# NVIDIA/cuopt

Measured on NVIDIA H100. Metric: pdlp_iterations_per_sec, higher is better.
Workload: dtype f64

## Files before the change

### cuopt_b200/csrc/pdlp_kernels.cuh

```cuda
#pragma once

#include "device_utils.cuh"
#include "spmv_bicsr.cuh"

#include <math_constants.h>

namespace cuopt_b200 {

constexpr int EW_THREADS  = 256;
static __device__ int g_l2_hints = 1;

struct pdhg_ctl_t {
  double step_size, primal_weight, tau, sigma;
  double pending_weight;
  double sum_weights;
  double interaction, norm_dx2, norm_dy2;
  double reduction_exponent, growth_exponent, primal_smoothing, dual_smoothing;
  int parity;
  int pending_avg;
  int active;
  int valid;
  int k_pdhg;
  int attempts;
  int accepted;
// ... 645 lines not shown
    dy2 += __ldcg(scal + 4 * g + 2);
  }
  pdhg_step_rule(ctl, interaction, dx2, dy2);
}

template <int FMT = 0>
__global__ void __launch_bounds__(BICSR_THREADS, BICSR_MIN_CTAS) k_block_pass(const pdhg_ctl_t* __restrict__ ctl,
                                                                              bicsr_view_t Ab,
                                                                              const double* __restrict__ x0,
                                                                              const double* __restrict__ x1,
                                                                              int pick_candidate,
                                                                              double* __restrict__ t,
                                                                              int first,
                                                                              const unsigned long long* wait_flags,
                                                                              int n_wait)
{
  if (!ctl->active) return;
  __shared__ double rows[BICSR_WARPS][BICSR_SLOTS];
  if (wait_flags) peer_wait(wait_flags, n_wait, (unsigned long long)ctl->attempts + 1ull);
  const double* x       = pick_candidate ? (ctl->parity ? x0 : x1) : x0;
  const l2_policy_t pol = make_l2_policies(g_l2_hints);
  struct payload_t {
    double init;
  };
  auto pre_op = [&](int r) {
    payload_t p;
    p.init = first ? 0.0 : ld_l2(t + r, pol.stream);
    return p;
  };
  auto row_op = [&](int r, double s, const payload_t&) { st_l2(t + r, s, pol.stream); };
  spmv_bicsr_rows<payload_t, true, 1, FMT>(Ab, x, rows[threadIdx.x >> 5], pre_op, row_op, pol.keep);
}

__global__ void __launch_bounds__(EW_THREADS) k_flush_average(const pdhg_ctl_t* __restrict__ ctl,
                                                              int n,
                                                              const double* __restrict__ xbuf0,
                                                              const double* __restrict__ xbuf1,
                                                              double* __restrict__ sum_x,
                                                              int m,
                                                              const double* __restrict__ ybuf0,
                                                              const double* __restrict__ ybuf1,
                                                              double* __restrict__ sum_y)
{
  if (!ctl->pending_avg) return;
  const int cur    = ctl->parity;
  const double* x  = cur ? xbuf1 : xbuf0;
  const double* y  = cur ? ybuf1 : ybuf0;
  const double w   = ctl->pending_weight;
  const int stride = gridDim.x * blockDim.x;
  for (int j = blockIdx.x * blockDim.x + threadIdx.x; j < n; j += stride) sum_x[j] = sum_x[j] + w * x[j];
  for (int i = blockIdx.x * blockDim.x + threadIdx.x; i < m; i += stride) sum_y[i] = sum_y[i] + w * y[i];
}
__global__ void k_clear_pending(pdhg_ctl_t* ctl) { ctl->pending_avg = 0; }
__global__ void k_begin_batch(pdhg_ctl_t* ctl, int steps)
{
  ctl->target = ctl->accepted + steps;
  ctl->valid  = 0;
  ctl->active = steps > 0 ? 1 : 0;
}

__global__ void __launch_bounds__(BICSR_THREADS, BICSR_MIN_CTAS) k_spmv(bicsr_view_t A,
                                                                        const double* __restrict__ x,
                                                                        double* __restrict__ out)
{
  __shared__ double rows[BICSR_WARPS][BICSR_SLOTS];
  struct payload_t {};
// ... 569 lines not shown
```

### cuopt_b200/csrc/pdlp_solver.cu

```cuda
#include "pdlp_solver.hpp"

#include "dist_comm.hpp"
#include "pdlp_kernels.cuh"
#include "presolve.cuh"
#include "trust_region.cuh"

#include <math_constants.h>
#include <nvtx3/nvToolsExt.h>

#include <algorithm>
#include <chrono>
#include <cmath>
#include <cstdio>
#include <cstdlib>
#include <atomic>
#include <map>
#include <mutex>
#include <thread>
#include <string>

namespace cuopt_b200 {

namespace {

// ... 31 lines not shown
    structure = &o;
    val.copy_from(o.val, s);
  }
};

constexpr int SCHEDULE_SEGMENT = 1 << 16;
template <typename T, typename F>
std::vector<T> cut_in_segments(int rows, F cut_segment)
{
  const int n_seg = std::max(1, (rows + SCHEDULE_SEGMENT - 1) / SCHEDULE_SEGMENT);
  std::vector<std::vector<T>> part(n_seg);
  const int n_thr = (int)std::max(1u, std::min<unsigned>({std::thread::hardware_concurrency(), 32u, (unsigned)n_seg}));
  std::atomic<int> next{0};
  auto work = [&]() {
    for (int sgm = next.fetch_add(1); sgm < n_seg; sgm = next.fetch_add(1))
      cut_segment(sgm * SCHEDULE_SEGMENT, std::min(rows, (sgm + 1) * SCHEDULE_SEGMENT), part[sgm]);
  };
  if (n_thr <= 1) {
    work();
  } else {
    std::vector<std::thread> pool;
    for (int t = 0; t < n_thr; ++t) pool.emplace_back(work);
    for (auto& t : pool) t.join();
  }
  size_t total = 0;
  for (auto& v : part) total += v.size();
  std::vector<T> all;
  all.reserve(total + 1);
  for (auto& v : part) all.insert(all.end(), v.begin(), v.end());
  return all;
}

template <typename VI>
void build_bicsr(csr_dev_t& d, const VI& off, cudaStream_t s, int sms)
{
  const int all_rows = (int)off.size() - 1;
  constexpr int LONG = (int)0x80000000u;
  std::vector<int2> cut = cut_in_segments<int2>(all_rows, [&](int r, int rows, std::vector<int2>& out) {
    while (r < rows) {
      const int lo = off[r];
      if (off[r + 1] - lo > BICSR_SLOTS) {
        out.push_back(make_int2(r | LONG, r + 1));
        ++r;
        continue;
      }
      int r1 = r;
      while (r1 < rows && off[r1 + 1] - lo <= BICSR_SLOTS && (r1 - r) < BICSR_MAX_ROWS) ++r1;
      out.push_back(make_int2(r, r1));
      r = r1;
    }
  });
  std::vector<int2> desc;
  desc.reserve(cut.size());
  for (const int2& c : cut)
    if (!(c.x & LONG)) desc.push_back(c);
  const int n_std = (int)desc.size();
  for (const int2& c : cut)
    if (c.x & LONG) desc.push_back(make_int2(c.x & ~LONG, c.y));
  bicsr_dev_t& b = d.bi;
  b.n_std        = n_std;
  b.n_blk        = (int)desc.size();
  b.desc.upload(desc, s);
  b.row_slot.resize((size_t)std::max(all_rows, 1));
  b.idx.resize((size_t)std::max(n_std, 1) * BICSR_SLOTS);
  b.val.resize((size_t)std::max(n_std, 1) * BICSR_SLOTS);
  if (all_rows > 0) CUOPT_CUDA_TRY(cudaMemsetAsync(b.row_slot.data(), 0xff, (size_t)all_rows * sizeof(unsigned short), s));
  if (n_std > 0) {
    const int grid = std::max(1, std::min((n_std + 7) / 8, sms * 8));
    k_bicsr_fill<<<grid, 256, 0, s>>>(n_std, b.desc.data(), d.off.data(), d.idx.data(), d.val.data(), b.idx.data(),
                                      b.val.data(), b.row_slot.data());
    CUOPT_CUDA_TRY(cudaGetLastError());
  }
}
void fill_bicsr_values(csr_dev_t& d, cudaStream_t s, int sms)
{
  const bicsr_dev_t& st = d.bi_structure();
  d.bi.val.resize((size_t)std::max(st.n_std, 1) * BICSR_SLOTS);
  if (st.n_std > 0) {
    const int grid = std::max(1, std::min((st.n_std + 7) / 8, sms * 8));
    k_bicsr_fill_values<<<grid, 256, 0, s>>>(st.n_std, st.desc.data(), d.off_ptr(), d.val.data(), d.bi.val.data());
    CUOPT_CUDA_TRY(cudaGetLastError());
  }
}

void compact_bicsr(csr_dev_t& d, int fmt, int col0, cudaStream_t s, int sms)
{
  bicsr_dev_t& b = d.bi;
  b.fmt  = fmt;
  b.col0 = col0;
  if (fmt == 0 || b.n_std == 0) return;
  const size_t ns = (size_t)b.n_std;
  if (fmt & BICSR_FMT_IDX3) {
    b.lo16.resize(ns * BICSR_SLOTS);
    b.hi8.resize(ns * 32);
  }
  if (fmt & BICSR_FMT_MASK) b.mask.resize(ns * 8);
  const int grid = std::max(1, std::min((b.n_std + BICSR_WARPS - 1) / BICSR_WARPS, sms * 8));
  k_bicsr_fill_structure<<<grid, BICSR_THREADS, 0, s>>>(b.n_std, b.desc.data(), d.off.data(), d.idx.data(), col0,
                                                        b.lo16.data(), b.hi8.data(), b.mask.data());
  CUOPT_CUDA_TRY(cudaGetLastError());
  CUOPT_CUDA_TRY(cudaStreamSynchronize(s));
  if (fmt & BICSR_FMT_IDX3) b.idx = dvec<int>{};
  if (fmt & BICSR_FMT_MASK) b.row_slot = dvec<unsigned short>{};
}

// ... 129 lines not shown
  cudaEvent_t free_[SLOTS] = {};
  bool ensure()
  {
    if (tried_) return buf_ != nullptr;
    tried_ = true;
    if (cudaMallocHost(&buf_, SLOT * SLOTS) != cudaSuccess) {
      cudaGetLastError();
      buf_ = nullptr;
      return false;
    }
    for (auto& e : free_) cudaEventCreateWithFlags(&e, cudaEventDisableTiming);
    return true;
  }
};
template <typename T, typename V>
void upload_staged(dvec<T>& d, const V& h, cudaStream_t s)
{
  d.resize(h.size());
  staged_uploader_t::get().upload(d.data(), h.data(), h.size() * sizeof(T), s);
}
template <typename VI, typename VD>
void upload_csr(csr_dev_t& d, int rows, int cols, const VI& off, const VI& idx, const VD& val, cudaStream_t s, int sms)
{
  d.rows = rows;
  d.cols = cols;
  d.nnz  = (int)val.size();
  upload_staged(d.off, off, s);
  upload_staged(d.idx, idx, s);
  upload_staged(d.val, val, s);
  build_bicsr(d, off, s, sms);
}

constexpr double GATHER_BLOCK_L2_FRACTION = 0.32;

}

struct pdlp_solver_t::impl_t {
  int m = 0, n = 0, nnz = 0;
  bool maximize    = false;
  double obj_scale = 1.0, obj_offset = 0.0;
  pdlp_hyper_params_t hp;
  pdlp_settings_t st;
  cudaStream_t stream = nullptr;
  int sms             = 132;

  csr_dev_t A, AT, As, ATs;
  dvec<double> c, l, u, lc, uc, cs, ls, us, lcs, ucs, Dr, Dc;
  dvec<double> xbuf[2], ybuf[2], atybuf[2], xbar, sum_x, sum_y, x_avg, y_avg, x_lr, y_lr, rc_cur, rc_avg;
  dvec<double> part_dy2, part_k3, part_rows, part_cols, part_misc, scratch_n, scratch_m, d_scalar;
  dvec<double> dist_buf;
  const dist_context_t* dist = nullptr;
  bool sharded() const { return dist != nullptr && dist->world > 1; }
  bool dist_gather = false;
  int row0[DIST_MAX_PEERS + 1] = {};
  int m_total = 0;
  dvec<double> yfull, t_slice;
  void* yfull_peer[DIST_MAX_PEERS] = {};
  peer_ptrs_t p_yfull{};
  csr_dev_t ATslice;
  csr_dev_t Ahot;
  dvec<int> sendX, sendY;
  dvec<int> listX, listY;
  send_plan_t planX{}, planY{};
  dvec<double> xloc;
  int cntX = 0, cntY = 0;
  bool dist_pack = true;
// ... 28 lines not shown
  void* scal_peer[DIST_MAX_PEERS]  = {};
  void* flag_peer[DIST_MAX_PEERS]  = {};
  bool peers_open = false;
  peer_ptrs_t p_xbar{}, p_scal{};
  peer_flags_t p_flags{};
  dvec<unsigned> d_ticket;
  dvec<pdhg_ctl_t> d_ctl;
  dvec<eval_t> d_eval;
  pdhg_ctl_t* h_ctl = nullptr;
  eval_t* h_eval    = nullptr;
  double* h_scalar  = nullptr;
  int occ_spmv = 1;
  int occ_spmv2 = 1;
  int npre_override = 0;
  int compact_blocks = BICSR_FMT_IDX3 | BICSR_FMT_MASK;
  dvec<double> eval_m, eval_n;
  dvec<double> part_max;
  dvec<double> part_infeas;
  bool tr_enabled = false;
  double tr_gap_reduction_last_trial = 1.0;
  int grid_tr = 1;
  dvec<double> tr_aty, tr_ax, tr_grad, tr_dir, tr_thr, tr_thr_sorted, tr_A, tr_B, tr_parts, tr_scal;
  dvec<int> tr_iota, tr_perm;
  struct tr_gap_t {
    const double *px, *py;
    double pd = 0, dd = 0, dist = 0, lower = 0, upper = 0, ngap = 0;
  };
  struct gather_blocks_t {
    int B = 1, width = 0;
    int fmt = 0;
    std::vector<csr_dev_t> blk;
    std::vector<csr_dev_t> unscaled;
    std::vector<int> grid;
    bool on() const { return B > 1; }
  };
  gather_blocks_t blkA, blkAT, blkATslice;
  dvec<double> t_m, t_n;
  size_t gather_block_bytes = 0;
  int n_part_dy2 = 1;
  int grid_k1 = 1, grid_k2 = 1, grid_k3 = 1, grid_n = 1, grid_m = 1, grid_misc = 1;
  long long staged_fills = 0;
  std::map<int, cudaGraphExec_t> graphs;
  bool use_graphs = true;
  cudaEvent_t ev_a = nullptr, ev_b = nullptr;

  int total_pdlp_iterations      = 0;
  bool initialised               = false;
  bool need_aty                  = true;
  bool last_restart_was_average  = false;
  bool warm_started              = false;
  double last_candidate_kkt      = 0.0, last_restart_kkt = 0.0;
  double l2_norm_b = 0.0, l2_norm_c = 0.0;
  lp_solution_t sol;
  bool finished   = false;
  bool presolved    = false;
  bool postsolved   = false;
  presolve_state_t ps;
  double t_start  = 0.0;
  long long launches = 0;

  void close_peer_memory(bool collective)
  {
    if (!peers_open) return;
    cudaStreamSynchronize(stream);
    dist->close_peers(xbar_peer);
    dist->close_peers(scal_peer);
    dist->close_peers(flag_peer);
    dist->close_peers(yfull_peer);
    peers_open = false;
    if (collective) {
      dist->allreduce(d_scalar.data(), 1, true, stream);
// ... 173 lines not shown
    size_t pad = 0;
    if (sharded()) {
      if (dist->world > DIST_MAX_PEERS) throw lp_error(error_type_t::ValidationError, "at most 8 ranks per solve");
      nslice   = (((n + dist->world - 1) / dist->world) + 31) & ~31;
      n_pad    = nslice * dist->world;
      slice_j0 = std::min(n, dist->rank * nslice);
      slice_n  = std::max(0, std::min(nslice, n - slice_j0));
      pad      = (size_t)(n_pad - n);
    }
    for (int b = 0; b < 2; ++b) {
      xbuf[b].resize(n, pad); xbuf[b].zero(stream);
      ybuf[b].resize(m); ybuf[b].zero(stream);
      atybuf[b].resize(n, pad); atybuf[b].zero(stream);
    }
    xbar.resize(n, pad + (sharded() ? 64 * (size_t)dist->world + 64 : 0));
    xbar.zero(stream);
    sum_x.resize(n, pad);
    sum_x.zero(stream);
    for (dvec<double>* v : {&x_avg, &x_lr, &rc_cur, &rc_avg, &scratch_n}) { v->resize(n); v->zero(stream); }
    for (dvec<double>* v : {&sum_y, &y_avg, &y_lr, &scratch_m}) { v->resize(m); v->zero(stream); }
    Dr.resize(m);
    Dc.resize(n);

    {
      int o2 = 1, o3 = 1;
      CUOPT_CUDA_TRY(cudaOccupancyMaxActiveBlocksPerMultiprocessor(&o2, (const void*)k_dual_step<true, 1>, BICSR_THREADS, 0));
      CUOPT_CUDA_TRY(cudaOccupancyMaxActiveBlocksPerMultiprocessor(&o3, (const void*)k_transpose_step<true, 1>, BICSR_THREADS, 0));
      occ_spmv = std::max(1, std::min(o2, o3));
      CUOPT_CUDA_TRY(cudaOccupancyMaxActiveBlocksPerMultiprocessor(&o2, (const void*)k_dual_step<true, 2>, BICSR_THREADS, 0));
      CUOPT_CUDA_TRY(cudaOccupancyMaxActiveBlocksPerMultiprocessor(&o3, (const void*)k_transpose_step<true, 2>, BICSR_THREADS, 0));
      occ_spmv2 = std::max(1, std::min(o2, o3));
      if (const char* e = std::getenv("CUOPT_B200_SPMV_NPRE")) npre_override = std::atoi(e);
    }
    grid_k2   = spmv_grid(As);
    grid_k3   = spmv_grid(ATs);
    grid_n    = ew_grid(n, sms);
    grid_m    = ew_grid(m, sms);
    grid_k1   = grid_n;
    grid_misc = ew_grid(std::max(n, m), sms);
    part_dy2.resize((size_t)std::max({grid_k2, grid_m, sms * 16}));
    n_part_dy2 = grid_k2;
    {
      int l2 = 0;
      CUOPT_CUDA_TRY(cudaDeviceGetAttribute(&l2, cudaDevAttrL2CacheSize, dev));
      gather_block_bytes = (size_t)((double)l2 * GATHER_BLOCK_L2_FRACTION);
    }
    if (const char* e = std::getenv("CUOPT_B200_GATHER_BLOCK_BYTES")) gather_block_bytes = (size_t)std::atoll(e);
    if (const char* e = std::getenv("CUOPT_B200_COMPACT_BLOCKS")) compact_blocks = std::atoi(e) & (BICSR_FMT_IDX3 | BICSR_FMT_MASK);
    part_k3.resize(2 * (size_t)std::max({grid_k3, grid_n, sms * 16}));
    part_rows.resize(6 * (size_t)grid_m);
    if (hp.restart_strategy == 2) {
      tr_enabled = true;
      {
        if (sharded())
          throw lp_error(error_type_t::ValidationError, "Methodical1 is not available in multi-GPU solves");
        const size_t N = (size_t)n + m;
        grid_tr        = ew_grid((int)std::min<size_t>(N, 1u << 30), sms);
        tr_aty.resize(n); tr_ax.resize(m); tr_grad.resize(N); tr_dir.resize(N); tr_thr.resize(N); tr_thr_sorted.resize(N);
        tr_A.resize(N); tr_B.resize(N); tr_iota.resize(N); tr_perm.resize(N);
        tr_parts.resize(5 * (size_t)grid_tr);
        tr_scal.resize(TR_SCALARS);
        tr_scal.zero(stream);
      }
    }
    if (st.detect_infeasibility) {
      if (sharded())
// ... 164 lines not shown
  }
  double initial_primal_weight(const dvec<double>& cc, const dvec<double>& lo, const dvec<double>& hi)
  {
    const double bn = std::sqrt(setup_reduce(2, m, lo.data(), hi.data(), hp.initial_primal_weight_b_scaling, true));
    const double cn = std::sqrt(setup_reduce(1, n, cc.data(), nullptr, hp.initial_primal_weight_c_scaling));
    return (bn > 0.0 && cn > 0.0) ? hp.primal_importance * (cn / bn) : hp.primal_importance;
  }

  void initialise()
  {
    if (initialised) return;
    nvtx_range_t nvtx_scope("pdlp initialise: scaling, initial step size / primal weight");
    const double t0 = now_seconds();
    trace.mark("(gap between build and initialise)");
    l2_norm_c = std::sqrt(setup_reduce(1, n, c.data(), nullptr, 1.0));
    l2_norm_b = std::sqrt(setup_reduce(2, m, lc.data(), uc.data(), 1.0, true));
    trace.mark("norms");
    compute_scaling_vectors();
    trace.mark("scaling vectors (Ruiz + Pock-Chambolle)");
    double step = 0.0, weight = 0.0;
    if (hp.compute_initial_step_size_before_scaling) step = initial_step_size(A);
    if (hp.compute_initial_primal_weight_before_scaling) weight = initial_primal_weight(c, lc, uc);
    scale_problem();
    fill_bicsr_values(As, stream, sms);
    fill_bicsr_values(ATs, stream, sms);
    trace.mark("scale problem + scaled BICSR values");
    if (dist_gather) {
      build_gather_transport();
    } else {
      build_gather_blocks(As, blkA, t_m, 0, sharded() ? nullptr : &A);
      build_gather_blocks(ATs, blkAT, t_n, 0, sharded() ? nullptr : &AT);
    }
    trace.mark("gather blocks");
    n_part_dy2 = k2_grid();
    if (!hp.compute_initial_step_size_before_scaling) step = initial_step_size(As);
    if (!hp.compute_initial_primal_weight_before_scaling) weight = initial_primal_weight(cs, lcs, ucs);

    pdhg_ctl_t k{};
    k.step_size          = step;
    k.primal_weight      = weight;
    k.tau                = step / weight;
    k.sigma              = step * weight;
    k.reduction_exponent = hp.reduction_exponent;
    k.growth_exponent    = hp.growth_exponent;
    k.primal_smoothing   = hp.primal_distance_smoothing;
    k.dual_smoothing     = hp.dual_distance_smoothing;
    *h_ctl               = k;
    if (st.warm_start && !st.warm_start->empty()) apply_warm_start(*st.warm_start);
    CUOPT_CUDA_TRY(cudaMemcpyAsync(d_ctl.data(), h_ctl, sizeof(k), cudaMemcpyHostToDevice, stream));
    if (hp.project_initial_primal) {
      k_clamp<<<grid_n, EW_THREADS, 0, stream>>>(n, xbuf[0].data(), ls.data(), us.data());
      k_clamp<<<grid_n, EW_THREADS, 0, stream>>>(n, x_avg.data(), ls.data(), us.data());
    }
    check_launch();
    sync();
    trace.mark("initial step size / primal weight, control block");
    sol.stats.initial_step_size     = step;
    sol.stats.initial_primal_weight = weight;
    sol.stats.setup_seconds += now_seconds() - t0;
    initialised = true;
  }

  void apply_warm_start(const pdlp_warm_start_t& w)
  {
    auto need = [&](const std::vector<double>& v, int size, const char* what) {
      if ((int)v.size() != size)
// ... 205 lines not shown
    trace.mark("  gather transport: xbar send tables and lists");
    std::vector<int> hoff = build_slice_transpose();
    trace.mark("  gather transport: rows J_g of the global A^T from the peers");
    const int WY = packed_positions(m_total, m_total, ATslice.nnz, ATslice.idx.data(), hy, posY);
    cntY         = 2 * WY;
    if ((size_t)cntY > yfull.size()) throw lp_error(error_type_t::RuntimeError, "gather transport: packed y' exceeds its buffer");
    if (ATslice.nnz > 0)
      k_remap_indices<<<ew_grid(ATslice.nnz, sms), EW_THREADS, 0, stream>>>(ATslice.nnz, ATslice.idx.data(), posY.data(),
                                                                            ATslice.idx.data());
    ATslice.cols = cntY;
    trace.mark("  gather transport: packed A^T slice (positions, renumbered indices)");
    build_gather_blocks(ATslice, blkATslice, t_slice, WY);
    if (!blkATslice.on()) build_bicsr(ATslice, hoff, stream, sms);
    trace.mark("  gather transport: column blocks of the A^T slice");
    exchange_positions(posY, row0[rk], m, sendY);
    build_send_lists(sendY, m, hy.half[rk], listY, planY);
    trace.mark("  gather transport: y' send tables and lists");
    check_launch();
    sync();
  }

  void build_gather_blocks(const csr_dev_t& M, gather_blocks_t& g, dvec<double>& t, int forced_width = 0,
                           const csr_dev_t* unscaled_src = nullptr)
  {
    g = gather_blocks_t{};
    const size_t bytes = (size_t)M.cols * sizeof(double);
    int B              = 1;
    if (forced_width > 0) {
      if (M.nnz == 0 || M.rows == 0) return;
      g.width = forced_width;
      B       = 2;
    } else {
      if (gather_block_bytes == 0 || bytes <= gather_block_bytes + gather_block_bytes / 2 || M.nnz == 0) return;
      B       = (int)std::min<size_t>(16, (bytes + gather_block_bytes - 1) / gather_block_bytes);
      g.width = (((M.cols + B - 1) / B) + 31) & ~31;
      B       = (M.cols + g.width - 1) / g.width;
    }
    if (B <= 1) return;
    g.B = B;
    if (forced_width == 0 && !sharded()) {
      g.fmt = compact_blocks;
      if (g.width > BICSR_IDX3_MAX_WIDTH) g.fmt &= ~BICSR_FMT_IDX3;
    }
    g.blk.resize(B);
    std::vector<int*> offs(B), idxs(B);
    std::vector<double*> vals(B);
    std::vector<int> nnz_b(B, 0);
    for (int b = 0; b < B; ++b) {
      g.blk[b].rows = M.rows;
      g.blk[b].cols = M.cols;
      g.blk[b].off.resize((size_t)M.rows + 1);
      offs[b] = g.blk[b].off.data();
    }
    csr_split_columns_offsets(M.rows, M.off_ptr(), M.idx_ptr(), g.width, B, offs.data(), nnz_b.data(), stream);
    for (int b = 0; b < B; ++b) {
      g.blk[b].nnz = nnz_b[b];
      g.blk[b].idx.resize((size_t)nnz_b[b]);
      g.blk[b].val.resize((size_t)nnz_b[b]);
      idxs[b] = g.blk[b].idx.data();
      vals[b] = g.blk[b].val.data();
    }
    csr_split_columns_fill(M.rows, M.off_ptr(), M.idx_ptr(), M.val.data(), g.width, B, offs.data(), idxs.data(), vals.data(),
                           stream);
    std::vector<int> hoff((size_t)M.rows + 1);
    g.grid.resize(B);
    for (int b = 0; b < B; ++b) {
      g.blk[b].off.download(hoff.data(), stream);
      sync();
      build_bicsr(g.blk[b], hoff, stream, sms);
      compact_bicsr(g.blk[b], g.fmt, b * g.width, stream, sms);
      g.grid[b] = spmv_grid(g.blk[b]);
    }
    if (unscaled_src) {
      g.unscaled.resize(B);
      for (int b = 0; b < B; ++b) {
        csr_dev_t& U = g.unscaled[b];
        U.rows = M.rows; U.cols = M.cols; U.nnz = nnz_b[b];
        U.structure = &g.blk[b];
        U.val.resize((size_t)nnz_b[b]);
        vals[b] = U.val.data();
      }
      csr_split_columns_fill(M.rows, M.off_ptr(), M.idx_ptr(), unscaled_src->val.data(), g.width, B, offs.data(), idxs.data(),
                             vals.data(), stream);
      for (csr_dev_t& U : g.unscaled) {
        fill_bicsr_values(U, stream, sms);
        if (U.bi_structure().n_std == U.bi_structure().n_blk) {
          sync();
          U.val = dvec<double>{};
        }
      }
    }
    t.resize((size_t)M.rows);
    t.zero(stream);
  }
  void launch_block_passes(const gather_blocks_t& g, int count, const double* x0, const double* x1, int pick_candidate,
                           double* t, const unsigned long long* wait_flags, int n_wait)
  {
    for (int b = 0; b < count; ++b) {
      const csr_dev_t& M = g.blk[b];
      with_fmt(g.fmt, [&](auto F) {
        k_block_pass<decltype(F)::value><<<g.grid[b], BICSR_THREADS, 0, stream>>>(
          d_ctl.data(), M.view(), x0, x1, pick_candidate, t, b == 0, b == 0 ? wait_flags : nullptr, n_wait);
      });
    }
  }
  void enqueue_k2(const unsigned long long* wait_flags, int n_wait, bool bcast = false,
                  const unsigned long long* wait_flags_b = nullptr)
  {
    const bool blocked  = blkA.on();
    const csr_dev_t& L  = blocked ? blkA.blk[blkA.B - 1] : hot_A();
    const int npre      = fused_npre(L);
    const int grid      = spmv_grid(L, npre);
    const double* t     = blocked ? t_m.data() : nullptr;
    const unsigned long long* wf = wait_flags_b ? wait_flags_b : (blocked ? nullptr : wait_flags);
    if (blocked) launch_block_passes(blkA, blkA.B - 1, xbar.data(), xbar.data(), 0, t_m.data(), wait_flags, n_wait);
#define CUOPT_K2(INIT, NPRE, FMT)                                                                                        \
  k_dual_step<INIT, NPRE, false, FMT><<<grid, BICSR_THREADS, 0, stream>>>(                                               \
    d_ctl.data(), L.view(), xbar.data(), ybuf[0].data(), ybuf[1].data(), lcs.data(), ucs.data(), sum_y.data(),          \
    part_dy2.data(), wf, n_wait, t)
#define CUOPT_K2B(INIT, NPRE)                                                                                            \
  k_dual_step<INIT, NPRE, true><<<grid, BICSR_THREADS, 0, stream>>>(d_ctl.data(), L.view(), xbar.data(), ybuf[0].data(), \
                                                                    ybuf[1].data(), lcs.data(), ucs.data(), sum_y.data(), \
                                                                    part_dy2.data(), wf, n_wait, t, p_yfull, p_flags,     \
                                                                    dist->world, dist->rank, sendY.data(), m)
    if (bcast) {
      if (blocked) { if (npre > 1) CUOPT_K2B(true, 2); else CUOPT_K2B(true, 1); }
      else { if (npre > 1) CUOPT_K2B(false, 2); else CUOPT_K2B(false, 1); }
    } else if (blocked) {
      with_fmt(blkA.fmt, [&](auto F) {
        if (npre > 1) CUOPT_K2(true, 2, decltype(F)::value); else CUOPT_K2(true, 1, decltype(F)::value);
      });
    } else { if (npre > 1) CUOPT_K2(false, 2, 0); else CUOPT_K2(false, 1, 0); }
#undef CUOPT_K2B
#undef CUOPT_K2
  }
  int k2_grid() const
  {
    const csr_dev_t& L = blkA.on() ? blkA.blk[blkA.B - 1] : hot_A();
    return spmv_grid(L, fused_npre(L));
  }
  int k3_npre() const { return npre_override > 1 ? 2 : 1; }
  int k3_grid() const { return spmv_grid(blkAT.on() ? blkAT.blk[blkAT.B - 1] : ATs, k3_npre()); }
  void enqueue_k3()
  {
    const bool blocked = blkAT.on();
    const csr_dev_t& L = blocked ? blkAT.blk[blkAT.B - 1] : ATs;
    const int npre     = k3_npre();
    const int grid     = k3_grid();
    const double* t    = blocked ? t_n.data() : nullptr;
    if (blocked) launch_block_passes(blkAT, blkAT.B - 1, ybuf[0].data(), ybuf[1].data(), 1, t_n.data(), nullptr, 0);
#define CUOPT_K3(INIT, NPRE, FMT)                                                                                         \
  k_transpose_step<INIT, NPRE, FMT><<<grid, BICSR_THREADS, 0, stream>>>(                                                  \
    d_ctl.data(), L.view(), ybuf[0].data(), ybuf[1].data(), xbuf[0].data(), xbuf[1].data(), atybuf[0].data(),            \
    atybuf[1].data(), part_k3.data(), part_dy2.data(), n_part_dy2, t)
    if (blocked) {
      with_fmt(blkAT.fmt, [&](auto F) {
        if (npre > 1) CUOPT_K3(true, 2, decltype(F)::value); else CUOPT_K3(true, 1, decltype(F)::value);
      });
    } else { if (npre > 1) CUOPT_K3(false, 2, 0); else CUOPT_K3(false, 1, 0); }
#undef CUOPT_K3
  }
  int kernels_per_attempt() const
  {
    const int k2 = blkA.on() ? blkA.B : 1;
    if (!sharded()) return 1 + k2 + (blkAT.on() ? blkAT.B : 1);
    if (dist_gather) return 1 + k2 + (blkATslice.on() ? blkATslice.B : 1) + 1 + (dist_send_kernel ? 2 : 0);
    return 1 + k2 + (blkAT.on() ? blkAT.B : 1) + 2;
  }

  void launch_transpose_partial()
  {
    if (blkAT.on()) {
      launch_block_passes(blkAT, blkAT.B, ybuf[0].data(), ybuf[1].data(), 1, dist_buf.data(), nullptr, 0);
      return;
    }
    k_transpose_partial<<<grid_k3, BICSR_THREADS, 0, stream>>>(d_ctl.data(), ATs.view(), ybuf[0].data(), ybuf[1].data(),
                                                               dist_buf.data());
  }
  void launch_spmv(const csr_dev_t& M, const double* v, double* out)
  {
    k_spmv<<<spmv_grid(M), BICSR_THREADS, 0, stream>>>(M.view(), v, out);
  }
  int launch_spmv_pair(const csr_dev_t& M, const gather_blocks_t& g, const double* u, const double* v, double* out_u,
                       double* out_v)
  {
    const int count = g.unscaled.empty() ? 1 : (int)g.unscaled.size();
    for (int b = 0; b < count; ++b) {
      const csr_dev_t& Mb = g.unscaled.empty() ? M : g.unscaled[b];
      with_fmt(g.fmt, [&](auto F) {
        k_spmv_pair<decltype(F)::value><<<spmv_grid(Mb), BICSR_THREADS, 0, stream>>>(Mb.view(), u, v, out_u, out_v, b == 0);
      });
    }
    return count;
  }

  void enqueue_sliced_attempt()
  {
    const int j0 = slice_j0, G = dist->world, rk = dist->rank;
// ... 78 lines not shown
      check_launch();
      return;
    }
    auto it = graphs.find(count);
    if (it == graphs.end()) {
      cudaGraph_t g;
      CUOPT_CUDA_TRY(cudaStreamBeginCapture(stream, cudaStreamCaptureModeThreadLocal));
      for (int i = 0; i < count; ++i) enqueue_attempt();
      CUOPT_CUDA_TRY(cudaStreamEndCapture(stream, &g));
      cudaGraphExec_t ge;
      CUOPT_CUDA_TRY(cudaGraphInstantiate(&ge, g, 0));
      cudaGraphDestroy(g);
      it = graphs.emplace(count, ge).first;
    }
    CUOPT_CUDA_TRY(cudaGraphLaunch(it->second, stream));
  }

  void fetch_ctl()
  {
    if (d_ctl.size() == 0) return;
    CUOPT_CUDA_TRY(cudaMemcpyAsync(h_ctl, d_ctl.data(), sizeof(pdhg_ctl_t), cudaMemcpyDeviceToHost, stream));
    sync();
  }

  void run_steps(int steps)
  {
    if (steps <= 0) return;
    nvtx_range_t nvtx_scope("take_step batch (PDHG attempts up to the next major iteration)");
    CUOPT_CUDA_TRY(cudaEventRecord(ev_a, stream));
    k_begin_batch<<<1, 1, 0, stream>>>(d_ctl.data(), steps);
    if (need_aty) {
      const int cur = h_ctl->parity;
      if (blkAT.on() && !sharded()) {
        launch_block_passes(blkAT, blkAT.B, ybuf[cur].data(), ybuf[cur].data(), 0, atybuf[cur].data(), nullptr, 0);
        launches += blkAT.B;
      } else {
        launch_spmv(ATs, ybuf[cur].data(), atybuf[cur].data());
        ++launches;
      }
      if (sharded()) dist->allreduce(atybuf[cur].data(), n, false, stream);
      need_aty = false;
    }
    const int target = h_ctl->accepted + steps;
    int todo         = steps;
    while (true) {
      launch_attempts(todo + (todo >= 16 ? 2 : 0));
      const int fj0 = sharded() ? slice_j0 : 0, fn = sharded() ? slice_n : n;
      k_flush_average<<<grid_misc, EW_THREADS, 0, stream>>>(d_ctl.data(), fn, xbuf[0].data() + fj0, xbuf[1].data() + fj0,
                                                            sum_x.data() + fj0, m, ybuf[0].data(), ybuf[1].data(),
                                                            sum_y.data());
      k_clear_pending<<<1, 1, 0, stream>>>(d_ctl.data());
      launches += 3;
      check_launch();
      fetch_ctl();
      if (h_ctl->valid == -1 || h_ctl->accepted >= target) break;
      todo = target - h_ctl->accepted;
    }
    if (sharded()) {
      const int cur = h_ctl->parity;
      dist->allgather(xbuf[cur].data(), nslice, stream);
      dist->allgather(atybuf[cur].data(), nslice, stream);
      dist->allgather(sum_x.data(), nslice, stream);
    }
    CUOPT_CUDA_TRY(cudaEventRecord(ev_b, stream));
    CUOPT_CUDA_TRY(cudaEventSynchronize(ev_b));
    float ms = 0.f;
    cudaEventElapsedTime(&ms, ev_a, ev_b);
    sol.stats.pdhg_loop_seconds += ms * 1e-3;
// ... 587 lines not shown
  s.t_start        = t0;
  s.outer_loop(-1);
  s.close_peer_memory(true);
  s.sol.stats.solve_time = now_seconds() - t0;
  return s.sol;
}

double pdlp_solver_t::scalar(const std::string& name)
{
  impl_t& s = *impl_;
  s.fetch_ctl();
  const pdhg_ctl_t& k = *s.h_ctl;
  if (name == "step_size") return k.step_size;
  if (name == "primal_weight") return k.primal_weight;
  if (name == "tau") return k.tau;
  if (name == "sigma") return k.sigma;
  if (name == "sum_w") return k.sum_weights;
  if (name == "k_total") return s.total_pdlp_iterations;
  if (name == "k_pdhg") return k.attempts;
  if (name == "its_since_restart") return k.its_since_restart;
  if (name == "interaction") return k.interaction;
  if (name == "norm_dx2") return k.norm_dx2;
  if (name == "norm_dy2") return k.norm_dy2;
  if (name == "l2_norm_b") return s.l2_norm_b;
  if (name == "l2_norm_c") return s.l2_norm_c;
  if (name == "last_restart_kkt") return s.last_restart_kkt;
  if (name == "last_candidate_kkt") return s.last_candidate_kkt;
  if (name == "n_restarts") return s.sol.stats.n_restarts;
  if (name == "last_restart_was_average") return s.last_restart_was_average ? 1.0 : 0.0;
  if (name == "eval_blocks") return (double)std::max<size_t>(1, s.blkA.unscaled.size());
  if (name == "eval_blocks_t") return (double)std::max<size_t>(1, s.blkAT.unscaled.size());
  if (name == "blocks_form_a") return s.blkA.fmt;
  if (name == "blocks_form_at") return s.blkAT.fmt;
  if (name == "valid") return k.valid;
  if (name == "sm_count") return s.sms;
  if (name == "occ_spmv") return s.occ_spmv;
  if (name == "occ_spmv2") return s.occ_spmv2;
  if (name == "grid_k1") return s.grid_k1;
  if (name == "grid_k2") return s.k2_grid();
  if (name == "grid_k3") return s.k3_grid();
  if (name == "grid_n") return s.grid_n;
  if (name == "grid_m") return s.grid_m;
  if (name == "k2_npre") return s.fused_npre(s.blkA.on() ? s.blkA.blk[s.blkA.B - 1] : s.hot_A());
  if (name == "n_std_a") return s.As.bi_structure().n_std;
  if (name == "n_blk_a") return s.As.bi_structure().n_blk;
  if (name == "n_std_at") return s.ATs.bi_structure().n_std;
  if (name == "n_blk_at") return s.ATs.bi_structure().n_blk;
  if (name == "staged_fills") return (double)s.staged_fills;
  if (name == "device_cache_hits") return (double)device_block_cache_t::get().hits();
  if (name == "presolve_offset") return s.ps.offset;
  return std::nan("");
}

std::vector<double> pdlp_solver_t::vector(const std::string& name)
{
  impl_t& s = *impl_;
  s.fetch_ctl();
  const int cur         = s.h_ctl->parity;
  const dvec<double>* v = nullptr;
  if (name == "x") v = &s.xbuf[cur];
  else if (name == "y") v = &s.ybuf[cur];
  else if (name == "aty") v = &s.atybuf[cur];
  else if (name == "x_next") v = &s.xbuf[cur ^ 1];
  else if (name == "y_next") v = &s.ybuf[cur ^ 1];
  else if (name == "aty_next") v = &s.atybuf[cur ^ 1];
  else if (name == "x_bar") v = &s.xbar;
// ... 155 lines not shown
```

### cuopt_b200/csrc/spmv_bicsr.cuh

```cuda
#pragma once

#include "device_utils.cuh"

namespace cuopt_b200 {

constexpr int BICSR_CH              = 8;
constexpr int BICSR_SLOTS           = 32 * BICSR_CH;
constexpr int BICSR_MAX_ROWS        = 256;
constexpr int BICSR_THREADS         = 256;
constexpr int BICSR_WARPS           = BICSR_THREADS / 32;
constexpr int BICSR_PAD             = 0x7fffffff;
constexpr unsigned short BICSR_EMPTY = 0xffff;
constexpr int BICSR_MIN_CTAS        = 4;
__host__ __device__ constexpr int bicsr_min_ctas(int npre) { return npre > 1 ? 3 : BICSR_MIN_CTAS; }

__host__ __device__ constexpr int bicsr_slot(int q) { return (q % BICSR_CH) * 32 + q / BICSR_CH; }

constexpr int BICSR_FMT_IDX3     = 1;
constexpr int BICSR_FMT_MASK     = 2;
constexpr int BICSR_IDX3_MAX_WIDTH = 1 << 21;
constexpr unsigned BICSR_HI_PAD  = 0x40u;
constexpr unsigned BICSR_HI_END  = 0x80u;

struct bicsr_view_t {
// ... 87 lines not shown
  return before;
}

template <bool MASK = false>
__device__ __forceinline__ void bicsr_block_row_sums(const double (&a)[BICSR_CH], const double (&g)[BICSR_CH], unsigned ends,
                                                     int lane, double* rsw, int before = 0)
{
  constexpr unsigned FULL = 0xffffffffu;
  double s = 0.0, head = 0.0;
  const int kf = ends ? __ffs(ends) - 1 : -1;
  int ord      = before;
#pragma unroll
  for (int k = 0; k < BICSR_CH; ++k) {
    s = __dadd_rn(s, __dmul_rn(a[k], g[k]));
    const bool e = (ends >> k) & 1u;
    if (e && k != kf) rsw[MASK ? ord : k * 32 + lane] = s;
    if constexpr (MASK) ord += e;
    head = (k == kf) ? s : head;
    s    = e ? 0.0 : s;
  }
  double tail  = s;
  double carry = __shfl_up_sync(FULL, tail, 1);
  if (lane == 0) carry = 0.0;
  unsigned pending = __ballot_sync(FULL, kf < 0);
  while (pending) {
    if (kf < 0) tail = carry + s;
    carry = __shfl_up_sync(FULL, tail, 1);
    if (lane == 0) carry = 0.0;
    pending &= pending << 1;
  }
  if (kf >= 0) rsw[MASK ? before : kf * 32 + lane] = carry + head;
}

template <typename P, bool INIT = false, int NPRE = 1, int FMT = 0, typename PreOp, typename RowOp>
__device__ __forceinline__ void spmv_bicsr_rows(const bicsr_view_t& A,
                                                const double* __restrict__ x,
                                                double* rsw,
                                                PreOp& pre_op,
                                                RowOp& row_op,
                                                unsigned long long gather_policy)
{
  constexpr bool MASK     = (FMT & BICSR_FMT_MASK) != 0;
  const int lane          = threadIdx.x & 31;
  const int gwarp         = blockIdx.x * BICSR_WARPS + (threadIdx.x >> 5);
  const int nwarps        = gridDim.x * BICSR_WARPS;
  const double* xg        = bicsr_gather_base<FMT>(A, x);
  bicsr_cols_t<FMT> c;
  if (gwarp < A.n_std) bicsr_load_cols<FMT>(A, gwarp, lane, c);
  for (int b = gwarp; b < A.n_std; b += nwarps) {
    const int2 d  = __ldg(A.desc + b);
    const int r0 = d.x, r1 = d.y;
    P pl[NPRE];
    unsigned short slot[NPRE];
    bicsr_mask_cursor_t mc{0u, 0};
#pragma unroll
    for (int q = 0; q < NPRE; ++q) {
      slot[q] = BICSR_EMPTY;
      if (r0 + lane + 32 * q < r1) {
        pl[q] = pre_op(r0 + lane + 32 * q);
        if constexpr (!MASK) slot[q] = __ldg(A.row_slot + r0 + lane + 32 * q);
      }
    }
    const size_t base = (size_t)b * BICSR_SLOTS + lane;
    double a[BICSR_CH], g[BICSR_CH];
#pragma unroll
    for (int k = 0; k < BICSR_CH; ++k) a[k] = ld_stream(A.val + base + k * 32);
#pragma unroll
    for (int k = 0; k < BICSR_CH; ++k) {
      const int col = bicsr_col<FMT>(c, k);
      g[k]          = col >= 0 ? ld_l2(xg + col, gather_policy) : 0.0;
    }
    if constexpr (MASK) mc.mw = lane < 8 ? __ldg(A.mask + (size_t)b * 8 + lane) : 0u;
    const unsigned ends = bicsr_ends<FMT>(c);
    if (b + nwarps < A.n_std) bicsr_load_cols<FMT>(A, b + nwarps, lane, c);
    bicsr_block_row_sums<MASK>(a, g, ends, lane, rsw, MASK ? bicsr_ends_before(ends, lane) : 0);
    __syncwarp();
#pragma unroll
    for (int q = 0; q < NPRE; ++q) {
      int src = slot[q] != BICSR_EMPTY ? (int)slot[q] : -1;
      if constexpr (MASK) src = mc.next(q, lane);
      if (r0 + lane + 32 * q < r1) {
        double sum = src >= 0 ? rsw[src] : 0.0;
        if constexpr (INIT) sum = pl[q].init + sum;
        row_op(r0 + lane + 32 * q, sum, pl[q]);
      }
    }
    for (int q = NPRE; 32 * q < r1 - r0; ++q) {
      const int r = r0 + 32 * q + lane;
      int src     = -1;
      if constexpr (MASK) src = mc.next(q, lane);
      if (r < r1) {
        const P p2 = pre_op(r);
        if constexpr (!MASK) {
          const unsigned short s2 = __ldg(A.row_slot + r);
          src                     = s2 != BICSR_EMPTY ? (int)s2 : -1;
        }
        double sum = src >= 0 ? rsw[src] : 0.0;
        if constexpr (INIT) sum = p2.init + sum;
        row_op(r, sum, p2);
      }
    }
    __syncwarp();
  }
  for (int b = A.n_std + gwarp; b < A.n_blk; b += nwarps) {
    const int row = __ldg(A.desc + b).x;
    const int lo = __ldg(A.off + row), hi = __ldg(A.off + row + 1);
    P pl;
    if (lane == 0) pl = pre_op(row);
    double acc = 0.0;
    for (int e = lo + lane; e < hi; e += 32) acc += ld_stream(A.cval + e) * ld_l2(x + ld_stream(A.cidx + e), gather_policy);
    acc = warp_sum(acc);
    if (lane == 0) {
      if constexpr (INIT) acc = pl.init + acc;
      row_op(row, acc, pl);
    }
  }
}

template <int FMT = 0, typename RowOp>
__device__ __forceinline__ void spmv_bicsr_rows_pair(const bicsr_view_t& A,
                                                     const double* __restrict__ u,
                                                     const double* __restrict__ v,
                                                     double* rsw_u,
                                                     double* rsw_v,
                                                     RowOp& row_op,
                                                     unsigned long long gather_policy)
{
  constexpr bool MASK = (FMT & BICSR_FMT_MASK) != 0;
  const int lane   = threadIdx.x & 31;
  const int gwarp  = blockIdx.x * BICSR_WARPS + (threadIdx.x >> 5);
  const int nwarps = gridDim.x * BICSR_WARPS;
  const double* ug = bicsr_gather_base<FMT>(A, u);
  const double* vg = bicsr_gather_base<FMT>(A, v);
  for (int b = gwarp; b < A.n_std; b += nwarps) {
    const int2 d      = __ldg(A.desc + b);
    const size_t base = (size_t)b * BICSR_SLOTS + lane;
    bicsr_cols_t<FMT> c;
    double a[BICSR_CH], gu[BICSR_CH], gv[BICSR_CH];
    bicsr_load_cols<FMT>(A, b, lane, c);
    bicsr_mask_cursor_t mc{0u, 0};
#pragma unroll
    for (int k = 0; k < BICSR_CH; ++k) a[k] = ld_stream(A.val + base + k * 32);
#pragma unroll
    for (int k = 0; k < BICSR_CH; ++k) {
      const int col = bicsr_col<FMT>(c, k);
      gu[k]         = col >= 0 ? ld_l2(ug + col, gather_policy) : 0.0;
      gv[k]         = col >= 0 ? ld_l2(vg + col, gather_policy) : 0.0;
    }
    const unsigned ends = bicsr_ends<FMT>(c);
// ... 140 lines not shown
```

Before: 399.2.

## Fuse column-block SpMV passes into a row-chunked shared-memory sweep kernel

Column-blocked SpMV used to launch one pass per block, and each pass read and wrote the partial-sum vector t in global memory. A new sweep kernel instead gives each CTA a chunk of rows, keeps their partial sums in dynamic shared memory, and walks several column blocks per launch using host-built per-chunk descriptor ranges. The goal is fewer kernel launches and less global round-tripping of t. The cost is large shared-memory use per CTA, which may reduce occupancy, plus __syncthreads barriers between blocks and possible load imbalance across chunks.

```diff
diff --git a/cuopt_b200/csrc/pdlp_kernels.cuh b/cuopt_b200/csrc/pdlp_kernels.cuh
--- a/cuopt_b200/csrc/pdlp_kernels.cuh
+++ b/cuopt_b200/csrc/pdlp_kernels.cuh
@@ -701,6 +701,55 @@
   spmv_bicsr_rows<payload_t, true, 1, FMT>(Ab, x, rows[threadIdx.x >> 5], pre_op, row_op, pol.keep);
 }
 
+constexpr int SWEEP_MAX_BLOCKS = 16;
+struct sweep_views_t {
+  bicsr_view_t v[SWEEP_MAX_BLOCKS];
+};
+template <int FMT = 0>
+__global__ void __launch_bounds__(BICSR_THREADS, BICSR_MIN_CTAS) k_block_sweep(const pdhg_ctl_t* __restrict__ ctl,
+                                                                               const sweep_views_t blks,
+                                                                               int b0,
+                                                                               int count,
+                                                                               const int2* __restrict__ tab,
+                                                                               int stride,
+                                                                               int rows,
+                                                                               int chunk_rows,
+                                                                               int n_chunks,
+                                                                               const double* __restrict__ x0,
+                                                                               const double* __restrict__ x1,
+                                                                               int pick_candidate,
+                                                                               double* __restrict__ t)
+{
+  if (!ctl->active) return;
+  __shared__ double rsw[BICSR_WARPS][BICSR_SLOTS];
+  extern __shared__ double sums[];
+  const double* x       = pick_candidate ? (ctl->parity ? x0 : x1) : x0;
+  const l2_policy_t pol = make_l2_policies(g_l2_hints);
+  const int w           = threadIdx.x >> 5;
+  struct payload_t {};
+  auto pre_op = [](int) { return payload_t{}; };
+  for (int k = blockIdx.x; k < n_chunks; k += gridDim.x) {
+    const int r0 = k * chunk_rows, nr = min(chunk_rows, rows - r0);
+    for (int i = threadIdx.x; i < nr; i += BICSR_THREADS) sums[i] = b0 ? ld_l2(t + r0 + i, pol.stream) : 0.0;
+    __syncthreads();
+    auto row_op = [&](int r, double s, const payload_t&) {
+      if ((unsigned)(r - r0) < (unsigned)nr) sums[r - r0] = sums[r - r0] + s;
+    };
+    for (int b = b0; b < b0 + count; ++b) {
+      const int2* e = tab + 2 * ((size_t)k * stride + b);
+      const int2 s  = __ldg(e);
+      spmv_bicsr_walk<payload_t, false, 1, FMT>(blks.v[b], bicsr_walk_t{s.x, s.y, 0, 0, w, BICSR_WARPS}, x, rsw[w], pre_op,
+                                               row_op, pol.keep);
+      const int2 l = __ldg(e + 1);
+      spmv_bicsr_walk<payload_t, false, 1, FMT>(blks.v[b], bicsr_walk_t{0, 0, l.x, l.y, w, BICSR_WARPS}, x, rsw[w], pre_op,
+                                               row_op, pol.keep);
+      __syncthreads();
+    }
+    for (int i = threadIdx.x; i < nr; i += BICSR_THREADS) st_l2(t + r0 + i, sums[i], pol.stream);
+    __syncthreads();
+  }
+}
+
 __global__ void __launch_bounds__(EW_THREADS) k_flush_average(const pdhg_ctl_t* __restrict__ ctl,
                                                               int n,
                                                               const double* __restrict__ xbuf0,
diff --git a/cuopt_b200/csrc/pdlp_solver.cu b/cuopt_b200/csrc/pdlp_solver.cu
--- a/cuopt_b200/csrc/pdlp_solver.cu
+++ b/cuopt_b200/csrc/pdlp_solver.cu
@@ -87,7 +87,7 @@
 }
 
 template <typename VI>
-void build_bicsr(csr_dev_t& d, const VI& off, cudaStream_t s, int sms)
+std::vector<int2> build_bicsr(csr_dev_t& d, const VI& off, cudaStream_t s, int sms)
 {
   const int all_rows = (int)off.size() - 1;
   constexpr int LONG = (int)0x80000000u;
@@ -126,6 +126,7 @@
                                       b.val.data(), b.row_slot.data());
     CUOPT_CUDA_TRY(cudaGetLastError());
   }
+  return desc;
 }
 void fill_bicsr_values(csr_dev_t& d, cudaStream_t s, int sms)
 {
@@ -321,6 +322,24 @@
 }
 
 constexpr double GATHER_BLOCK_L2_FRACTION = 0.32;
+
+void sweep_chunk_ranges(const std::vector<int2>& desc, int n_std, int rows, int chunk_rows, int n_chunks, int b, int B,
+                        std::vector<int2>& tab)
+{
+  const int n_blk = (int)desc.size();
+  int s_lo = 0, s_hi = 0, l_lo = n_std, l_hi = n_std;
+  for (int k = 0; k < n_chunks; ++k) {
+    const int r0 = k * chunk_rows, r1 = std::min(rows, r0 + chunk_rows);
+    while (s_lo < n_std && desc[s_lo].y <= r0) ++s_lo;
+    s_hi = std::max(s_hi, s_lo);
+    while (s_hi < n_std && desc[s_hi].x < r1) ++s_hi;
+    while (l_lo < n_blk && desc[l_lo].x < r0) ++l_lo;
+    l_hi = std::max(l_hi, l_lo);
+    while (l_hi < n_blk && desc[l_hi].x < r1) ++l_hi;
+    tab[2 * ((size_t)k * B + b)]     = make_int2(s_lo, s_hi);
+    tab[2 * ((size_t)k * B + b) + 1] = make_int2(l_lo, l_hi);
+  }
+}
 
 }
 
@@ -415,11 +434,20 @@
     std::vector<csr_dev_t> blk;
     std::vector<csr_dev_t> unscaled;
     std::vector<int> grid;
+    int chunk_rows = 0, chunks = 0, sweep_grid = 0;
+    dvec<int2> tab;
+    sweep_views_t views{};
+    std::vector<std::vector<int2>> desc_host;
     bool on() const { return B > 1; }
+    bool sweeps() const { return chunks > 0; }
   };
   gather_blocks_t blkA, blkAT, blkATslice;
   dvec<double> t_m, t_n;
   size_t gather_block_bytes = 0;
+  bool block_sweep = true;
+  int sweep_capacity = 1;
+  int sweep_rows_forced = 0;
+  int sweep_group = 2;
   int n_part_dy2 = 1;
   int grid_k1 = 1, grid_k2 = 1, grid_k3 = 1, grid_n = 1, grid_m = 1, grid_misc = 1;
   long long staged_fills = 0;
@@ -659,6 +687,22 @@
       occ_spmv2 = std::max(1, std::min(o2, o3));
       if (const char* e = std::getenv("CUOPT_B200_SPMV_NPRE")) npre_override = std::atoi(e);
     }
+    {
+      int smem_sm = 0, reserved = 0;
+      CUOPT_CUDA_TRY(cudaDeviceGetAttribute(&smem_sm, cudaDevAttrMaxSharedMemoryPerMultiprocessor, dev));
+      CUOPT_CUDA_TRY(cudaDeviceGetAttribute(&reserved, cudaDevAttrReservedSharedMemoryPerBlock, dev));
+      const int bytes = smem_sm / BICSR_MIN_CTAS - reserved - (int)(sizeof(double) * BICSR_WARPS * BICSR_SLOTS);
+      sweep_capacity  = std::max(1, bytes / (int)sizeof(double));
+      for (int f = 0; f <= (BICSR_FMT_IDX3 | BICSR_FMT_MASK); ++f)
+        with_fmt(f, [&](auto F) {
+          const void* k = (const void*)k_block_sweep<decltype(F)::value>;
+          CUOPT_CUDA_TRY(cudaFuncSetAttribute(k, cudaFuncAttributeMaxDynamicSharedMemorySize, sweep_capacity * (int)sizeof(double)));
+          CUOPT_CUDA_TRY(cudaFuncSetAttribute(k, cudaFuncAttributePreferredSharedMemoryCarveout, cudaSharedmemCarveoutMaxShared));
+        });
+      if (const char* e = std::getenv("CUOPT_B200_BLOCK_SWEEP")) block_sweep = std::atoi(e) != 0;
+      if (const char* e = std::getenv("CUOPT_B200_SWEEP_ROWS")) sweep_rows_forced = std::max(0, std::atoi(e));
+      if (const char* e = std::getenv("CUOPT_B200_SWEEP_GROUP")) sweep_group = std::max(1, std::atoi(e));
+    }
     grid_k2   = spmv_grid(As);
     grid_k3   = spmv_grid(ATs);
     grid_n    = ew_grid(n, sms);
@@ -889,6 +933,11 @@
       build_gather_blocks(ATs, blkAT, t_n, 0, sharded() ? nullptr : &AT);
     }
     trace.mark("gather blocks");
+    if (block_sweep && !sharded()) {
+      build_sweep(blkA);
+      build_sweep(blkAT);
+      trace.mark("block sweep chunk tables");
+    }
     n_part_dy2 = k2_grid();
     if (!hp.compute_initial_step_size_before_scaling) step = initial_step_size(As);
     if (!hp.compute_initial_primal_weight_before_scaling) weight = initial_primal_weight(cs, lcs, ucs);
@@ -1160,7 +1209,7 @@
       B       = 2;
     } else {
       if (gather_block_bytes == 0 || bytes <= gather_block_bytes + gather_block_bytes / 2 || M.nnz == 0) return;
-      B       = (int)std::min<size_t>(16, (bytes + gather_block_bytes - 1) / gather_block_bytes);
+      B       = (int)std::min<size_t>(SWEEP_MAX_BLOCKS, (bytes + gather_block_bytes - 1) / gather_block_bytes);
       g.width = (((M.cols + B - 1) / B) + 31) & ~31;
       B       = (M.cols + g.width - 1) / g.width;
     }
@@ -1192,10 +1241,13 @@
                            stream);
     std::vector<int> hoff((size_t)M.rows + 1);
     g.grid.resize(B);
+    const bool swept = block_sweep && forced_width == 0 && !sharded();
+    if (swept) g.desc_host.resize(B);
     for (int b = 0; b < B; ++b) {
       g.blk[b].off.download(hoff.data(), stream);
       sync();
-      build_bicsr(g.blk[b], hoff, stream, sms);
+      std::vector<int2> desc = build_bicsr(g.blk[b], hoff, stream, sms);
+      if (swept) g.desc_host[b] = std::move(desc);
       compact_bicsr(g.blk[b], g.fmt, b * g.width, stream, sms);
       g.grid[b] = spmv_grid(g.blk[b]);
     }
@@ -1221,6 +1273,45 @@
     t.resize((size_t)M.rows);
     t.zero(stream);
   }
+  void build_sweep(gather_blocks_t& g)
+  {
+    if (!g.on()) return;
+    const int rows = g.blk[0].rows;
+    int occ        = 1;
+    with_fmt(g.fmt, [&](auto F) {
+      CUOPT_CUDA_TRY(cudaOccupancyMaxActiveBlocksPerMultiprocessor(&occ, (const void*)k_block_sweep<decltype(F)::value>,
+                                                                   BICSR_THREADS, sweep_capacity * sizeof(double)));
+    });
+    const long long wave = (long long)sms * std::max(1, occ);
+    if (sweep_rows_forced > 0) {
+      g.chunk_rows = std::min(sweep_rows_forced, sweep_capacity);
+    } else {
+      const long long W = (rows + wave * sweep_capacity - 1) / (wave * sweep_capacity);
+      g.chunk_rows      = (int)((rows + wave * W - 1) / (wave * W));
+    }
+    g.chunks     = (rows + g.chunk_rows - 1) / g.chunk_rows;
+    g.sweep_grid = (int)std::min<long long>(wave, g.chunks);
+    std::vector<int2> tab(2 * (size_t)g.chunks * g.B);
+    for (int b = 0; b < g.B; ++b) {
+      sweep_chunk_ranges(g.desc_host[b], g.blk[b].bi.n_std, rows, g.chunk_rows, g.chunks, b, g.B, tab);
+      g.views.v[b] = g.blk[b].view();
+    }
+    g.tab.upload(tab, stream);
+    sync();
+    g.desc_host.clear();
+  }
+  int sweep_launches(int count) const { return (count + sweep_group - 1) / sweep_group; }
+  void launch_block_sweep(const gather_blocks_t& g, int count, const double* x0, const double* x1, int pick_candidate,
+                          double* t)
+  {
+    for (int b0 = 0; b0 < count; b0 += sweep_group) {
+      with_fmt(g.fmt, [&](auto F) {
+        k_block_sweep<decltype(F)::value><<<g.sweep_grid, BICSR_THREADS, (size_t)g.chunk_rows * sizeof(double), stream>>>(
+          d_ctl.data(), g.views, b0, std::min(sweep_group, count - b0), g.tab.data(), g.B, g.blk[0].rows, g.chunk_rows,
+          g.chunks, x0, x1, pick_candidate, t);
+      });
+    }
+  }
   void launch_block_passes(const gather_blocks_t& g, int count, const double* x0, const double* x1, int pick_candidate,
                            double* t, const unsigned long long* wait_flags, int n_wait)
   {
@@ -1241,7 +1332,8 @@
     const int grid      = spmv_grid(L, npre);
     const double* t     = blocked ? t_m.data() : nullptr;
     const unsigned long long* wf = wait_flags_b ? wait_flags_b : (blocked ? nullptr : wait_flags);
-    if (blocked) launch_block_passes(blkA, blkA.B - 1, xbar.data(), xbar.data(), 0, t_m.data(), wait_flags, n_wait);
+    if (blocked && blkA.sweeps()) launch_block_sweep(blkA, blkA.B - 1, xbar.data(), xbar.data(), 0, t_m.data());
+    else if (blocked) launch_block_passes(blkA, blkA.B - 1, xbar.data(), xbar.data(), 0, t_m.data(), wait_flags, n_wait);
 #define CUOPT_K2(INIT, NPRE, FMT)                                                                                        \
   k_dual_step<INIT, NPRE, false, FMT><<<grid, BICSR_THREADS, 0, stream>>>(                                               \
     d_ctl.data(), L.view(), xbar.data(), ybuf[0].data(), ybuf[1].data(), lcs.data(), ucs.data(), sum_y.data(),          \
@@ -1276,7 +1368,8 @@
     const int npre     = k3_npre();
     const int grid     = k3_grid();
     const double* t    = blocked ? t_n.data() : nullptr;
-    if (blocked) launch_block_passes(blkAT, blkAT.B - 1, ybuf[0].data(), ybuf[1].data(), 1, t_n.data(), nullptr, 0);
+    if (blocked && blkAT.sweeps()) launch_block_sweep(blkAT, blkAT.B - 1, ybuf[0].data(), ybuf[1].data(), 1, t_n.data());
+    else if (blocked) launch_block_passes(blkAT, blkAT.B - 1, ybuf[0].data(), ybuf[1].data(), 1, t_n.data(), nullptr, 0);
 #define CUOPT_K3(INIT, NPRE, FMT)                                                                                         \
   k_transpose_step<INIT, NPRE, FMT><<<grid, BICSR_THREADS, 0, stream>>>(                                                  \
     d_ctl.data(), L.view(), ybuf[0].data(), ybuf[1].data(), xbuf[0].data(), xbuf[1].data(), atybuf[0].data(),            \
@@ -1290,8 +1383,8 @@
   }
   int kernels_per_attempt() const
   {
-    const int k2 = blkA.on() ? blkA.B : 1;
-    if (!sharded()) return 1 + k2 + (blkAT.on() ? blkAT.B : 1);
+    const int k2 = blkA.on() ? (blkA.sweeps() ? 1 + sweep_launches(blkA.B - 1) : blkA.B) : 1;
+    if (!sharded()) return 1 + k2 + (blkAT.on() ? (blkAT.sweeps() ? 1 + sweep_launches(blkAT.B - 1) : blkAT.B) : 1);
     if (dist_gather) return 1 + k2 + (blkATslice.on() ? blkATslice.B : 1) + 1 + (dist_send_kernel ? 2 : 0);
     return 1 + k2 + (blkAT.on() ? blkAT.B : 1) + 2;
   }
@@ -1436,8 +1529,13 @@
     if (need_aty) {
       const int cur = h_ctl->parity;
       if (blkAT.on() && !sharded()) {
-        launch_block_passes(blkAT, blkAT.B, ybuf[cur].data(), ybuf[cur].data(), 0, atybuf[cur].data(), nullptr, 0);
-        launches += blkAT.B;
+        if (blkAT.sweeps()) {
+          launch_block_sweep(blkAT, blkAT.B, ybuf[cur].data(), ybuf[cur].data(), 0, atybuf[cur].data());
+          launches += sweep_launches(blkAT.B);
+        } else {
+          launch_block_passes(blkAT, blkAT.B, ybuf[cur].data(), ybuf[cur].data(), 0, atybuf[cur].data(), nullptr, 0);
+          launches += blkAT.B;
+        }
       } else {
         launch_spmv(ATs, ybuf[cur].data(), atybuf[cur].data());
         ++launches;
@@ -2091,6 +2189,12 @@
   if (name == "eval_blocks_t") return (double)std::max<size_t>(1, s.blkAT.unscaled.size());
   if (name == "blocks_form_a") return s.blkA.fmt;
   if (name == "blocks_form_at") return s.blkAT.fmt;
+  if (name == "sweep_rows") return s.blkA.chunk_rows;
+  if (name == "sweep_chunks") return s.blkA.chunks;
+  if (name == "sweep_grid") return s.blkA.sweep_grid;
+  if (name == "sweep_rows_t") return s.blkAT.chunk_rows;
+  if (name == "sweep_chunks_t") return s.blkAT.chunks;
+  if (name == "sweep_grid_t") return s.blkAT.sweep_grid;
   if (name == "valid") return k.valid;
   if (name == "sm_count") return s.sms;
   if (name == "occ_spmv") return s.occ_spmv;
diff --git a/cuopt_b200/csrc/spmv_bicsr.cuh b/cuopt_b200/csrc/spmv_bicsr.cuh
--- a/cuopt_b200/csrc/spmv_bicsr.cuh
+++ b/cuopt_b200/csrc/spmv_bicsr.cuh
@@ -143,8 +143,17 @@
   if (kf >= 0) rsw[MASK ? before : kf * 32 + lane] = carry + head;
 }
 
+struct bicsr_walk_t {
+  int std_lo, std_hi, long_lo, long_hi, warp, nwarps;
+};
+__device__ __forceinline__ bicsr_walk_t bicsr_grid_walk(const bicsr_view_t& A)
+{
+  return {0, A.n_std, A.n_std, A.n_blk, (int)(blockIdx.x * BICSR_WARPS + (threadIdx.x >> 5)), (int)(gridDim.x * BICSR_WARPS)};
+}
+
 template <typename P, bool INIT = false, int NPRE = 1, int FMT = 0, typename PreOp, typename RowOp>
-__device__ __forceinline__ void spmv_bicsr_rows(const bicsr_view_t& A,
+__device__ __forceinline__ void spmv_bicsr_walk(const bicsr_view_t& A,
+                                                const bicsr_walk_t& wk,
                                                 const double* __restrict__ x,
                                                 double* rsw,
                                                 PreOp& pre_op,
@@ -153,12 +162,11 @@
 {
   constexpr bool MASK     = (FMT & BICSR_FMT_MASK) != 0;
   const int lane          = threadIdx.x & 31;
-  const int gwarp         = blockIdx.x * BICSR_WARPS + (threadIdx.x >> 5);
-  const int nwarps        = gridDim.x * BICSR_WARPS;
+  const int nwarps        = wk.nwarps;
   const double* xg        = bicsr_gather_base<FMT>(A, x);
   bicsr_cols_t<FMT> c;
-  if (gwarp < A.n_std) bicsr_load_cols<FMT>(A, gwarp, lane, c);
-  for (int b = gwarp; b < A.n_std; b += nwarps) {
+  if (wk.std_lo + wk.warp < wk.std_hi) bicsr_load_cols<FMT>(A, wk.std_lo + wk.warp, lane, c);
+  for (int b = wk.std_lo + wk.warp; b < wk.std_hi; b += nwarps) {
     const int2 d  = __ldg(A.desc + b);
     const int r0 = d.x, r1 = d.y;
     P pl[NPRE];
@@ -183,7 +191,7 @@
     }
     if constexpr (MASK) mc.mw = lane < 8 ? __ldg(A.mask + (size_t)b * 8 + lane) : 0u;
     const unsigned ends = bicsr_ends<FMT>(c);
-    if (b + nwarps < A.n_std) bicsr_load_cols<FMT>(A, b + nwarps, lane, c);
+    if (b + nwarps < wk.std_hi) bicsr_load_cols<FMT>(A, b + nwarps, lane, c);
     bicsr_block_row_sums<MASK>(a, g, ends, lane, rsw, MASK ? bicsr_ends_before(ends, lane) : 0);
     __syncwarp();
 #pragma unroll
@@ -213,7 +221,7 @@
     }
     __syncwarp();
   }
-  for (int b = A.n_std + gwarp; b < A.n_blk; b += nwarps) {
+  for (int b = wk.long_lo + wk.warp; b < wk.long_hi; b += nwarps) {
     const int row = __ldg(A.desc + b).x;
     const int lo = __ldg(A.off + row), hi = __ldg(A.off + row + 1);
     P pl;
@@ -226,6 +234,16 @@
       row_op(row, acc, pl);
     }
   }
+}
+template <typename P, bool INIT = false, int NPRE = 1, int FMT = 0, typename PreOp, typename RowOp>
+__device__ __forceinline__ void spmv_bicsr_rows(const bicsr_view_t& A,
+                                                const double* __restrict__ x,
+                                                double* rsw,
+                                                PreOp& pre_op,
+                                                RowOp& row_op,
+                                                unsigned long long gather_policy)
+{
+  spmv_bicsr_walk<P, INIT, NPRE, FMT>(A, bicsr_grid_walk(A), x, rsw, pre_op, row_op, gather_policy);
 }
 
 template <int FMT = 0, typename RowOp>
```

Result: slower. 250.4 (median of 6 runs) (-37.3%).
